# GatorSense/HyperPRI

Measured on AMD Instinct MI355X. Metric: HSI cubes/sec (608x968x238) fwd+bwd, higher is better.
Workload: dtype f32; 1 GPU; CubeNET-64 n_channels=238 HSI 608x968 fp32, per-GPU batch 2, train mode, BCEWithLogits, fwd+bwd; global_batch=2, parallelism=dp1

## Files before the change

### hyperpri_amd/csrc/api.cpp

```cpp
#include "common.h"
#include <string.h>

static thread_local char g_err[256] = "";

int hpri_set_error(int code, const char* msg) {
  strncpy(g_err, msg ? msg : "", sizeof(g_err) - 1);
  g_err[sizeof(g_err) - 1] = 0;
  return code;
}

extern "C" const char* hpri_last_error(void) { return g_err; }
extern "C" int hpri_version(void) { return 100; }

#include <stdlib.h>
#include <atomic>
#include <mutex>
static std::atomic<int> g_opt[8];
static std::once_flag g_opt_once;
static const char* const g_opt_name[8] = {"conv_nbx_min", "wgrad_xcd_min_tiles", "wgrad_xcd_min_strips", "bf16v3_tile_width", "bn_wide_cq", "wgrad_cu_reserve", "wgrad_skip_edge", "wino4_fast_epilogue"};
static const char* const g_opt_env[8] = {"HPRI_NBX_MIN", "HPRI_WGRAD_XCD_MIN", "HPRI_WGRAD_XCD_STRIPS", "HPRI_V3_TILE_WIDTH", "HPRI_BN_WIDE_CQ", "HPRI_WGRAD_CU_RESERVE", "HPRI_WGRAD_SKIP_EDGE", "HPRI_WINO4_FAST_EPILOGUE"};
static const int g_opt_default[8] = {9, 128, 2048, 0, 1, 0, 1, 1};

static void opt_init() {
  for (int i = 0; i < 8; ++i) {
    const char* e = getenv(g_opt_env[i]);
    int v = e ? atoi(e) : g_opt_default[i];
    if (v < 0) v = g_opt_default[i];
    g_opt[i].store(v, std::memory_order_relaxed);
  }
}

int hpri_option(int idx) {
  std::call_once(g_opt_once, opt_init);
  return g_opt[idx].load(std::memory_order_relaxed);
}

extern "C" int hpri_set_option(const char* name, int value) {
  std::call_once(g_opt_once, opt_init);
  for (int i = 0; i < 8; ++i)
    if (name && strcmp(name, g_opt_name[i]) == 0) {
      if (value < 0) return hpri_set_error(HPRI_ERR_ARG, "set_option: value must be >= 0");
      g_opt[i].store(value, std::memory_order_release);
      return HPRI_OK;
    }
  return hpri_set_error(HPRI_ERR_ARG, "set_option: unknown option");
}

static std::atomic<int> g_cus[16];
int hpri_cu_count() {
  int dev = 0;
  if (hipGetDevice(&dev) != hipSuccess || dev < 0 || dev >= 16) return 256;
  int n = g_cus[dev].load(std::memory_order_relaxed);
  if (n > 0) return n;
  if (hipDeviceGetAttribute(&n, hipDeviceAttributeMultiprocessorCount, dev) != hipSuccess || n <= 0) n = 256;
  g_cus[dev].store(n, std::memory_order_relaxed);
  return n;
}

static std::mutex g_q_mutex;
static struct { hipStream_t stream; unsigned* q; unsigned seq; bool used; } g_q[32];

HpriQueueHalves hpri_item_queue_take(hipStream_t stream) {
  std::lock_guard<std::mutex> lock(g_q_mutex);
  for (auto& e : g_q)
// ... 18 lines not shown
  if (queue == nullptr) return HPRI_OK;
  for (auto& e : g_q)
    if (!e.used) { e.stream = stream; e.q = reinterpret_cast<unsigned*>(queue); e.seq = 0; e.used = true; return HPRI_OK; }
  return hpri_set_error(HPRI_ERR_ARG, "set_item_queue: more than 32 streams hold a queue");
}

static thread_local float g_loss_scale = 1.f;
float hpri_loss_scale() { return g_loss_scale; }
extern "C" int hpri_set_loss_scale(float scale) {
  HPRI_REQUIRE(scale > 0.f, "set_loss_scale: the scale must be positive");
  g_loss_scale = scale;
  return HPRI_OK;
}

extern "C" int hpri_get_option(const char* name) {
  for (int i = 0; i < 8; ++i)
    if (name && strcmp(name, g_opt_name[i]) == 0) return hpri_option(i);
  return hpri_set_error(HPRI_ERR_ARG, "get_option: unknown option");
}
```

### hyperpri_amd/csrc/gemm_f32v2.hip

```cpp
#include "common.h"

#define F2_BN 128
#define F2_KC 16
#define F2_A_BYTES (256 * 64)
#define F2_B_BYTES (F2_BN * 64)
#define F2_STAGE_BYTES (F2_A_BYTES + F2_B_BYTES)

struct GemmF2Args {
  const float* x; int x_cs, x_coff;
  const float* wp;
  const float* bias;
  float* y; int y_cs, y_coff, y_cw;
  int N, HW;
  int W, H2, W2, py0, px0, cup;
  int nchunks, Ncols, Ncols_pad;
  int accumulate;
  int tiles_img, ntiles, nb_count, per_xcd;
  int ncu, stagger_cycles;
  unsigned *queue, *queue_clear;
};

struct F2Tile { int img, p0, valid, nb, bx; };

template <int MODE>
__global__ __launch_bounds__(256, 2) void gemm_f32v2_kernel(GemmF2Args a) {
  __shared__ __attribute__((aligned(1024))) unsigned char smem[3 * F2_STAGE_BYTES + 2 * F2_BN * 4 + 16];
  float* bias_lds = reinterpret_cast<float*>(smem + 3 * F2_STAGE_BYTES);
  int* next_lds = reinterpret_cast<int*>(smem + 3 * F2_STAGE_BYTES + 2 * F2_BN * 4);

  const int tid = threadIdx.x, lane = tid & 63, wave = __builtin_amdgcn_readfirstlane(tid >> 6);
  const int li = lane & 31, lh = lane >> 5;
  const int xcd = blockIdx.x & 7, nloc = (int)(gridDim.x >> 3);
  const int items_all = a.ntiles * a.nb_count;
  auto tile_of = [&](int k, F2Tile& t) -> bool {
    if (k >= a.per_xcd) return false;
    const int item = xcd * a.per_xcd + k;
    if (item >= items_all) return false;
    t.bx = item / a.nb_count; t.nb = item - t.bx * a.nb_count;
    t.img = t.bx / a.tiles_img;
    t.p0 = (t.bx - t.img * a.tiles_img) * 256;
    t.valid = min(256, a.HW - t.p0);
    return true;
  };

  constexpr unsigned OOB = HPRI_DMA_OOB;
  unsigned aoff[4], goff[2];
  hpri_rsrc_t rs_a = HPRI_MAKE_RSRC(a.x, 0x7FFFFF00);
  const hpri_rsrc_t rs_b = HPRI_MAKE_RSRC(a.wp, 0x7FFFFF00);
  const int chunk_bytes = a.Ncols_pad * 64;
  const int cpt = MODE == 2 ? (a.cup >> 4) : 1;
  auto setup_dma = [&](const F2Tile& t) {
#pragma unroll
    for (int q = 0; q < 4; ++q) {
      const int pix = (q * 4 + wave) * 16 + (lane >> 2);
      const unsigned sw = (unsigned)(((lane & 3) ^ ((pix >> 2) & 3)) << 2);
      unsigned off = OOB;
// ... 31 lines not shown
  __builtin_amdgcn_sched_barrier(0)
#define F2_DMA_A_AT(bo_, c_, q_) HPRI_LDS_DMA16(rs_a, smem + (bo_) + ((q_) * 4 + wave) * 1024, aoff[q_], a_soff(c_))
#define F2_DMA_B_AT(bo_, c_, q_) HPRI_LDS_DMA16(rs_b, smem + (bo_) + F2_A_BYTES + ((q_) * 4 + wave) * 1024, goff[q_], (c_) * chunk_bytes)
#define F2_ISSUE(buf_, c_)                                                               \
  {                                                                                      \
    _Pragma("unroll") for (int q = 0; q < 2; ++q) F2_DMA_B_AT((buf_) * F2_STAGE_BYTES, c_, q); \
    _Pragma("unroll") for (int q = 0; q < 4; ++q) F2_DMA_A_AT((buf_) * F2_STAGE_BYTES, c_, q); \
  }

  const int fofs0 = li * 64 + (((2 * lh + 0) ^ ((li >> 2) & 3)) << 4);
  const int fofs1 = li * 64 + (((2 * lh + 1) ^ ((li >> 2) & 3)) << 4);
  const int S = a.nchunks;

  F2Tile cur, nxt;
  int k = (int)(blockIdx.x >> 3);
  unsigned* const q = a.queue;
  if (blockIdx.x == 0) hpri_q_clear(a.queue_clear, tid);
  const int nstatic = min(nloc, a.ncu >> 3);
  const bool late_start = (unsigned)(blockIdx.x - a.ncu) < (unsigned)a.ncu;
  unsigned pend = 0u;
  if (q != nullptr && tid == 0) pend = hpri_q_draw(q, xcd, k < nstatic ? 1u : 2u);
  if (late_start && a.stagger_cycles > 0) {
    const long long t0 = (long long)__builtin_amdgcn_s_memtime();
    while ((long long)__builtin_amdgcn_s_memtime() - t0 < (long long)a.stagger_cycles) __builtin_amdgcn_s_sleep(32);
  }
  if (q != nullptr && k >= nstatic) {
    if (tid == 0) { next_lds[0] = nstatic + (int)pend; pend += 1u; }
    __syncthreads();
    k = __builtin_amdgcn_readfirstlane(next_lds[0]);
    __syncthreads();
  }
  bool have = tile_of(k, cur);
  if (!have) return;
  setup_dma(cur);
  float bias_next = 0.f;
  auto load_bias = [&](const F2Tile& t) {
    if (tid < F2_BN) {
      const int col = t.nb * F2_BN + tid;
      const int ch = MODE == 1 ? col % a.cup : col;
      bias_next = (a.bias != nullptr && col < a.Ncols) ? a.bias[ch] : 0.f;
    }
  };
  load_bias(cur);
  F2_ISSUE(0, 0)
  if (S > 1) F2_ISSUE(1, 1)
  int slot = 0;

  while (have) {
    if (tid < F2_BN) bias_lds[slot * F2_BN + tid] = bias_next;
    if (q != nullptr && tid == 0) next_lds[slot] = nstatic + (int)pend;

    f32x16 acc[4][2];
#pragma unroll
    for (int ct = 0; ct < 4; ++ct)
#pragma unroll
      for (int pt = 0; pt < 2; ++pt)
#pragma unroll
        for (int r = 0; r < 16; ++r) acc[ct][pt][r] = 0.f;

    int bo = 0;
    for (int s = 0; s < S; ++s) {
      if (s + 1 < S) F2_WAIT_VM(6); else F2_WAIT_VM(0);
      F2_BARRIER();
      const unsigned char* wb_ = smem + bo + F2_A_BYTES;
      const unsigned char* xb_ = smem + bo + wave * 4096;
      f32x4 wa[4][2], xb[2][2];
#pragma unroll
      for (int ct = 0; ct < 4; ++ct) {
        wa[ct][0] = *reinterpret_cast<const f32x4*>(wb_ + ct * 2048 + fofs0);
        wa[ct][1] = *reinterpret_cast<const f32x4*>(wb_ + ct * 2048 + fofs1);
      }
#pragma unroll
      for (int pt = 0; pt < 2; ++pt) {
        xb[pt][0] = *reinterpret_cast<const f32x4*>(xb_ + pt * 2048 + fofs0);
        xb[pt][1] = *reinterpret_cast<const f32x4*>(xb_ + pt * 2048 + fofs1);
      }
      const bool more_ = s + 2 < S;
      const int bo2 = bo == 0 ? 2 * F2_STAGE_BYTES : bo - F2_STAGE_BYTES;
      __builtin_amdgcn_s_setprio(1);
#pragma unroll
      for (int g = 0; g < 2; ++g)
#pragma unroll
        for (int j = 0; j < 4; ++j) {
#pragma unroll
          for (int ct = 0; ct < 4; ++ct)
#pragma unroll
            for (int pt = 0; pt < 2; ++pt)
              acc[ct][pt] = __builtin_amdgcn_mfma_f32_32x32x2f32(wa[ct][g][j], xb[pt][g][j], acc[ct][pt], 0, 0, 0);
          const int step = g * 4 + j;
          if (more_ && step < 2) { F2_DMA_B_AT(bo2, s + 2, step); }
          if (more_ && step >= 2 && step < 6) { F2_DMA_A_AT(bo2, s + 2, step - 2); }
        }
      __builtin_amdgcn_s_setprio(0);
      bo = bo == 2 * F2_STAGE_BYTES ? 0 : bo + F2_STAGE_BYTES;
    }
    F2_BARRIER();
    if (q != nullptr) k = __builtin_amdgcn_readfirstlane(next_lds[slot]);
    else k += nloc;
    have = tile_of(k, nxt);
    if (have) {
      setup_dma(nxt);
      F2_ISSUE(0, 0)
      if (S > 1) F2_ISSUE(1, 1)
      load_bias(nxt);
      if (q != nullptr && tid == 0) pend = hpri_q_draw(q, xcd, 1u);
    }

#pragma unroll
    for (int pt = 0; pt < 2; ++pt) {
      const int pix = wave * 64 + pt * 32 + li;
      const bool ok = pix < cur.valid;
      const int p = cur.p0 + min(pix, cur.valid - 1);
      long long orow;
      if (MODE == 1) {
        const int yy = p / a.W, xx = p - yy * a.W;
        orow = ((long long)cur.img * a.H2 + a.py0 + 2 * yy) * a.W2 + a.px0 + 2 * xx;
      } else {
        orow = (long long)cur.img * a.HW + p;
      }
      if (MODE != 1 && a.accumulate) {
#pragma unroll
        for (int hh = 0; hh < 2; ++hh) {
// ... 27 lines not shown
          if (MODE == 1) {
            if (ok && col < a.Ncols) {
              const int tap = col / a.cup, co = col - tap * a.cup;
              const long long rr = orow + (long long)((tap >> 1) * a.W2 + (tap & 1));
              *reinterpret_cast<f32x4*>(a.y + rr * a.y_cs + a.y_coff + co) = v;
            }
          } else {
            if (ok && col < a.y_cw) {
#pragma unroll
              for (int e = 0; e < 4; ++e) if (col + e >= a.Ncols) v[e] = 0.f;
              *reinterpret_cast<f32x4*>(a.y + orow * a.y_cs + a.y_coff + col) = v;
            }
          }
        }
    }
    cur = nxt;
    slot ^= 1;
  }
#undef F2_ISSUE
#undef F2_DMA_A_AT
#undef F2_DMA_B_AT
#undef F2_WAIT_VM
#undef F2_BARRIER
}

__global__ void pack_weight_f32k16_kernel(const float* __restrict__ w, float* __restrict__ wp, int mode, int K, int Ncols,
                                          int Ncols_pad, int chunks, int Cup, int src_d1) {
  const size_t total = (size_t)chunks * Ncols_pad * 16;
  for (size_t idx = (size_t)blockIdx.x * blockDim.x + threadIdx.x; idx < total; idx += (size_t)gridDim.x * blockDim.x) {
    const int kk = (int)(idx & 15);
    const size_t r = idx >> 4;
    const int col = (int)(r % Ncols_pad), chunk = (int)(r / Ncols_pad);
    const int k = chunk * 16 + kk;
    float v = 0.f;
    if (k < K && col < Ncols) {
      if (mode == 0) v = w[(size_t)col * src_d1 + k];
      else if (mode == 1) v = w[(size_t)k * src_d1 + col];
      else if (mode == 2) { const int tap = col / Cup, co = col - tap * Cup; v = w[((size_t)k * Cup + co) * 4 + tap]; }
// ... 9 lines not shown
                                       hipStream_t stream) {
  HPRI_REQUIRE(w && wp, "pack_weight_f32k16: null pointer");
  HPRI_REQUIRE(mode >= 0 && mode <= 3 && K > 0 && Ncols > 0 && Ncols_pad >= Ncols && Ncols_pad % 64 == 0, "pack_weight_f32k16: bad arguments");
  HPRI_REQUIRE(mode < 2 || Cup > 0, "pack_weight_f32k16: the transposed-convolution modes need Cup");
  const int chunks = hpri_cdiv(K, 16);
  const size_t total = (size_t)chunks * Ncols_pad * 16;
  int blocks = (int)((total + 255) / 256);
  if (blocks > 4096) blocks = 4096;
  hipLaunchKernelGGL(pack_weight_f32k16_kernel, dim3(blocks), dim3(256), 0, stream, w, wp, mode, K, Ncols, Ncols_pad, chunks, Cup, src_d1);
  HPRI_CHECK_LAUNCH();
  return HPRI_OK;
}

#define F2_STAGGER_CYCLES 8000

static int f2_launch(int mode, const float* x, int x_cs, int x_coff, const float* wp, const float* bias, float* y, int y_cs, int y_coff,
                     int y_cw, int N, long long HW, int W, int H2, int W2, int py0, int px0, int cup, int K_pad, int Ncols,
                     int Ncols_pad, int accumulate, hipStream_t stream) {
  HPRI_REQUIRE(x && wp && y, "gemm_f32v2: null pointer");
  HPRI_REQUIRE(N > 0 && HW > 0 && HW < (1ll << 30), "gemm_f32v2: bad row counts");
  HPRI_REQUIRE(K_pad > 0 && K_pad % 16 == 0, "gemm_f32v2: K_pad must be a positive multiple of 16");
  HPRI_REQUIRE(Ncols > 0 && Ncols_pad % 64 == 0 && Ncols <= Ncols_pad, "gemm_f32v2: Ncols_pad must be a multiple of 64 >= Ncols");
  HPRI_REQUIRE(x_cs % 4 == 0 && x_coff % 4 == 0 && x_cs > 0 && x_cs <= 16384, "gemm_f32v2: row stride / offset must be multiples of 4 (stride <= 16384)");
  HPRI_REQUIRE(((uintptr_t)x & 15) == 0 && ((uintptr_t)wp & 15) == 0 && ((uintptr_t)y & 15) == 0, "gemm_f32v2: pointers must be 16-byte aligned");
  HPRI_REQUIRE(y_cs % 4 == 0 && y_coff % 4 == 0, "gemm_f32v2: the output view must be float4-aligned");
  HPRI_REQUIRE((long long)(K_pad / 16) * Ncols_pad * 64 < 0x7FFFFF00ll, "gemm_f32v2: packed weights exceed 2 GiB");
  GemmF2Args a;
  a.x = x; a.x_cs = x_cs; a.x_coff = x_coff; a.wp = wp; a.bias = bias;
  a.y = y; a.y_cs = y_cs; a.y_coff = y_coff; a.y_cw = y_cw;
  a.N = N; a.HW = (int)HW; a.W = W; a.H2 = H2; a.W2 = W2; a.py0 = py0; a.px0 = px0; a.cup = cup;
  a.nchunks = K_pad / 16; a.Ncols = Ncols; a.Ncols_pad = Ncols_pad; a.accumulate = accumulate & 1;
  if (mode == 0 || mode == 2) {
    HPRI_REQUIRE(y_cw % 4 == 0 && y_cw >= Ncols && y_cw + y_coff <= y_cs, "gemm_f32v2: written width must be a multiple of 4 >= Ncols inside the row stride");
// ... 7 lines not shown
  }
  if (mode == 1) {
    HPRI_REQUIRE(cup % 4 == 0 && Ncols == 4 * cup && !a.accumulate, "gemm_f32v2: depth-to-space needs Cup % 4 == 0, 4*Cup columns and no accumulate");
    HPRI_REQUIRE(x_coff + K_pad <= x_cs && cup + y_coff <= y_cs, "gemm_f32v2: rows narrower than K_pad / Cup channels exceed the output stride");
  }
  if (mode == 2) {
    HPRI_REQUIRE(cup % 16 == 0 && K_pad == 4 * cup && x_coff + cup <= x_cs, "gemm_f32v2: space-to-depth needs Cup % 16 == 0 and K = 4*Cup");
    HPRI_REQUIRE((long long)H2 * W2 * x_cs * 4 < 0x7FFFFF00ll, "gemm_f32v2: one image of the gradient tensor exceeds 2 GiB (32-bit DMA offsets)");
  }
  a.tiles_img = (int)((HW + 255) / 256); a.ntiles = N * a.tiles_img; a.nb_count = (Ncols_pad + F2_BN - 1) / F2_BN;
  const long long items = (long long)a.ntiles * a.nb_count;
  HPRI_REQUIRE(items < (1ll << 28), "gemm_f32v2: too many work items");
  a.per_xcd = (int)((items + 7) / 8);
  a.ncu = hpri_cu_count(); a.stagger_cycles = F2_STAGGER_CYCLES;
  a.queue = a.queue_clear = nullptr;
  int nloc = (2 * a.ncu) / 8;
  if (nloc < 1) nloc = 1;
  if (nloc > a.per_xcd) nloc = a.per_xcd;
  dim3 grid((unsigned)(nloc * 8));
  if (a.per_xcd >= 2 * nloc) { const HpriQueueHalves qh = hpri_item_queue_take(stream); a.queue = qh.use; a.queue_clear = qh.clear; }
  if (mode == 0) hipLaunchKernelGGL(gemm_f32v2_kernel<0>, grid, dim3(256), 0, stream, a);
  else if (mode == 1) hipLaunchKernelGGL(gemm_f32v2_kernel<1>, grid, dim3(256), 0, stream, a);
  else hipLaunchKernelGGL(gemm_f32v2_kernel<2>, grid, dim3(256), 0, stream, a);
  HPRI_CHECK_LAUNCH();
  return HPRI_OK;
}

extern "C" int hpri_gemm_f32v2(const float* x, int x_cs, int x_coff, const float* wp, const float* bias, float* y, int y_cs, int y_coff,
                               int N, long long HW, int K_pad, int Ncols, int Ncols_pad, int y_cw, int accumulate, hipStream_t stream) {
  return f2_launch(0, x, x_cs, x_coff, wp, bias, y, y_cs, y_coff, y_cw, N, HW, 0, 0, 0, 0, 0, 0, K_pad, Ncols, Ncols_pad, accumulate, stream);
}

extern "C" int hpri_convt_fwd_f32v2(const float* x, int x_cs, int x_coff, const float* wp, const float* bias, float* y, int y_cs,
                                    int y_coff, int N, int H, int W, int K_pad, int Cup, int Ncols_pad, int H2, int W2, int py0, int px0,
                                    hipStream_t stream) {
  return f2_launch(1, x, x_cs, x_coff, wp, bias, y, y_cs, y_coff, 0, N, (long long)H * W, W, H2, W2, py0, px0, Cup, K_pad, 4 * Cup, Ncols_pad,
                   0, stream);
}

extern "C" int hpri_convt_dgrad_f32v2(const float* dy, int dy_cs, int dy_coff, const float* wp, float* dx, int dx_cs, int dx_coff, int N,
                                      int H, int W, int Cup, int Cin, int Cin_pad, int dx_cw, int H2, int W2, int py0, int px0,
                                      int accumulate, hipStream_t stream) {
  return f2_launch(2, dy, dy_cs, dy_coff, wp, nullptr, dx, dx_cs, dx_coff, dx_cw, N, (long long)H * W, W, H2, W2, py0, px0, Cup, 4 * Cup, Cin,
                   Cin_pad, accumulate & 1, stream);
}
```

### hyperpri_amd/engine.py

```python
from __future__ import annotations

import contextlib
import ctypes
import threading
import os
import types
from typing import Callable, Dict, List, Optional, Tuple

import torch

from . import _lib

A_DIRECT, A_S2D = 0, 1
E_DIRECT, E_D2S = 0, 1

PRECISIONS = ("fp32", "bf16", "bf16x3", "bf16x6")
LOWP = ("bf16", "bf16x3", "bf16x6")
_SPLIT = {"bf16": 0, "bf16x3": 1, "bf16x6": 2}
DEFAULT_PRECISION = os.environ.get("HPRI_PRECISION", "fp32")

TORCH = "torch"
_CALL = threading.local()


# ... 781 lines not shown
def _pack(w: torch.Tensor, mode: int, K: int, ncols: int, T: int, cup: int, d1: int) -> Tuple[torch.Tensor, int]:
    ncols_pad = _rup(ncols, 64)

    def build():
        global PACK_LAUNCHES
        n = _lib.load().hpri_packed_weight_floats(K, ncols_pad, T)
        wp = torch.empty(n, dtype=torch.float32, device=w.device)
        _lib.call("hpri_pack_weight", _p(w), _p(wp), mode, K, ncols, ncols_pad, T, cup, 0, d1, _stream())
        PACK_LAUNCHES += 1
        return wp
    return _cached_pack(w, ("f32", mode, K, ncols, T, cup, d1), build), ncols_pad


GEMM_F32V2 = True
GEMM_F32V2_DGRAD = False


def _pack_f32k16(w: torch.Tensor, mode: int, K: int, ncols: int, cup: int, d1: int = 0) -> Tuple[torch.Tensor, int]:
    ncols_pad = _rup(ncols, 64)

    def build():
        global PACK_LAUNCHES
        wp = torch.empty(_lib.load().hpri_packed_weight_f32k16_floats(K, ncols_pad), dtype=torch.float32, device=w.device)
        _lib.call("hpri_pack_weight_f32k16", _p(w), _p(wp), mode, K, ncols, ncols_pad, cup, d1, _stream())
        PACK_LAUNCHES += 1
        return wp
    return _cached_pack(w, ("f32k16", mode, K, ncols, cup, d1), build), ncols_pad


def _pack_bf16(w: torch.Tensor, mode: int, K: int, ncols: int, T: int, d1: int, cup: int = 0,
# ... 874 lines not shown
            with _timed("gemm_planes_bf16<convT,s2d>", 2.0 * x1.N * x1.H * x1.W * cin * 4 * cup):
                _lib.call("hpri_convt_dgrad_bf16v3_y16", _p(gpl.buf), gpl.cs, gpl.coff, _p(wpd), gx.ptr, gx.cs, gx.coff, x1.N, x1.H, x1.W,
                          cup, cin, cols_pad, cin, H2, W2, py0, px0, _stream())
        else:
            gx, acc = tp.grad_slot(x1)
            with _timed("gemm_planes_bf16<convT,s2d>", 2.0 * x1.N * x1.H * x1.W * cin * 4 * cup):
                _lib.call("hpri_convt_dgrad_bf16v3", _p(gpl.buf), gpl.cs, gpl.coff, _p(wpd), gx.ptr, gx.cs, gx.coff, x1.N, x1.H, x1.W, cup,
                          cin, cols_pad, gx.cw, H2, W2, py0, px0, int(acc), _stream())
    elif need_dx1:
        gx, acc = tp.grad_slot(x1)
        if bprec in LOWP:
            wpd, cols_pad = _pack_bf16(weight, 3, 4 * cup, cin, 1, cup, cup, split=_SPLIT.get(bprec, 0))
            _conv_launch_bf16(gu, wpd, None, gx, None, x1.N, x1.H, x1.W, 4 * cup, cin, cols_pad, gx.cw, 1,
                              amode=A_S2D, accumulate=int(acc), H2=H2, W2=W2, py0=py0, px0=px0, cup=cup, cin_true=4 * cup,
                              split=_SPLIT.get(bprec, 0))
        elif GEMM_F32V2_DGRAD and cup % 16 == 0 and H2 * W2 * gu.cs * 4 < 0x7FFFFF00 and x1.N * H2 * W2 < (1 << 31):
            wpd, cols_pad = _pack_f32k16(weight, 3, 4 * cup, cin, cup)
            with _timed("gemm_f32v2<convT,s2d>", 2.0 * x1.N * x1.H * x1.W * cin * 4 * cup):
                _lib.call("hpri_convt_dgrad_f32v2", gu.ptr, gu.cs, gu.coff, _p(wpd), gx.ptr, gx.cs, gx.coff, x1.N, x1.H, x1.W, cup, cin, cols_pad,
                          gx.cw, H2, W2, py0, px0, int(acc), _stream())
        else:
            wpd, cols_pad = _pack(weight, 3, 4 * cup, cin, 1, cup, cup)
            _conv_launch(gu, wpd, None, gx, None, x1.N, x1.H, x1.W, 4 * cup, cin, cols_pad, gx.cw, 1,
                         amode=A_S2D, accumulate=int(acc), H2=H2, W2=W2, py0=py0, px0=px0, cup=cup, cin_true=4 * cup)


def _upsample_into(tape: Tape, x1: Act, dst: Act, weight: Optional[torch.Tensor], bias: Optional[torch.Tensor],
                   need_dx1: bool, precision: Optional[str] = None, dst_planes=None) -> bool:
    dev = x1.buf.device
    H2, W2 = dst.H, dst.W
    dY, dX = H2 - 2 * x1.H, W2 - 2 * x1.W
    py0, px0 = dY // 2, dX // 2
    cup = dst.C
    if cup % 4:
        raise RuntimeError("hyperpri_amd: Up: channel counts must be multiples of 4")
    if dY < 0 or dX < 0:
        full = Act.new(x1.N, 2 * x1.H, 2 * x1.W, cup, dev)
        _upsample_into(tape, x1, full, weight, bias, need_dx1, precision)
        _lib.call("hpri_shift_copy", full.ptr, full.cs, full.coff, full.H, full.W, dst.ptr, dst.cs, dst.coff, dst.N, H2, W2,
# ... 31 lines not shown
                              px0 + 2 * x1.W, _stream())
                with _timed("gemm_planes_bf16<convT,d2s+planes>", 2.0 * x1.N * x1.H * x1.W * cin * 4 * cup):
                    _lib.call("hpri_convt_fwd_bf16v3", _p(xp_.buf), xp_.cs, xp_.coff, _p(wp), _p(bias), ctypes.c_void_p(0), 0, 0,
                              _p(pl.buf), pl.cs, pc0, x1.N, x1.H, x1.W, _rup(cin, 32), cup, ncols_pad, H2, W2, py0, px0, _stream())
            else:
                with _timed("conv_fwd_bf16<1,4x1,direct,d2s+planes>", 2.0 * x1.N * x1.H * x1.W * cin * 4 * cup):
                    _lib.call("hpri_convt_fwd_bf16_pl", x1.ptr, x1.cs, x1.coff, _p(wp), _p(bias), ctypes.c_void_p(0), dst.cs, dst.coff,
                              x1.N, x1.H, x1.W, x1.cw, 4 * cup, ncols_pad, H2, W2, py0, px0, cup, _p(pl.buf), pl.cs, pc0, _stream())
            planes_written = True
        elif bf16:
            wp, ncols_pad = _pack_bf16(weight, 2, cin, 4 * cup, 1, cup, cup, split=usplit)
            _conv_launch_bf16(x1, wp, bias, dst, None, x1.N, x1.H, x1.W, x1.cw, 4 * cup, ncols_pad, 4 * cup, 1,
                              epi=E_D2S, H2=H2, W2=W2, py0=py0, px0=px0, cup=cup, cin_true=cin, split=usplit)
        elif GEMM_F32V2 and cin % 16 == 0 and x1.N * H2 * W2 < (1 << 31):
            wp, ncols_pad = _pack_f32k16(weight, 2, cin, 4 * cup, cup)
            with _timed("gemm_f32v2<convT,d2s>", 2.0 * x1.N * x1.H * x1.W * cin * 4 * cup):
                _lib.call("hpri_convt_fwd_f32v2", x1.ptr, x1.cs, x1.coff, _p(wp), _p(bias), dst.ptr, dst.cs, dst.coff, x1.N, x1.H, x1.W, cin,
                          cup, ncols_pad, H2, W2, py0, px0, _stream())
        else:
            wp, ncols_pad = _pack(weight, 2, cin, 4 * cup, 1, cup, cup)
            _conv_launch(x1, wp, bias, dst, None, x1.N, x1.H, x1.W, x1.cw, 4 * cup, ncols_pad, 4 * cup, 1,
                         epi=E_D2S, H2=H2, W2=W2, py0=py0, px0=px0, cup=cup, cin_true=cin)
        del wp
    else:
        if x1.C != cup:
            raise RuntimeError("hyperpri_amd: Up: bilinear upsampling keeps the channel count")
        _lib.call("hpri_upsample2x_fwd", x1.ptr, x1.cs, x1.coff, dst.ptr, dst.cs, dst.coff, x1.N, x1.H, x1.W, H2, W2,
                  py0, px0, cup, _stream())
    if not tape.record:
        return planes_written
    c = types.SimpleNamespace(dst=dst, weight=weight, bias=bias, need_dx1=need_dx1, x1=x1, precision=precision, dev=dev, H2=H2, W2=W2,
                              py0=py0, px0=px0, cup=cup, dY=dY, dX=dX)
    tape.note_params(weight, bias)
# ... 337 lines not shown
```

### include/hyperpri_hip.h

```cpp
#ifndef HYPERPRI_HIP_H
#define HYPERPRI_HIP_H

#include <stddef.h>
#include <hip/hip_runtime_api.h>

#ifdef __cplusplus
extern "C" {
#endif

#define HPRI_OK 0
#define HPRI_ERR_ARG (-1)
#define HPRI_ERR_UNSUPPORTED (-2)
#define HPRI_ERR_WORKSPACE (-3)
#define HPRI_ERR_LAUNCH (-4)

#define HPRI_A_DIRECT 0
#define HPRI_A_S2D 1
#define HPRI_E_DIRECT 0
#define HPRI_E_D2S 1

int hpri_version(void);
int hpri_set_option(const char* name, int value);


// ... 90 lines not shown
                        float* stats, int N, int H, int W, int Cin_pad, int Cout, int Cout_pad, int y_cw, void* y2, int y2_cs,
                        int y2_coff, int y2_c0, int y2_cw, int y2_only, hipStream_t stream);


size_t hpri_packed_weight_f32k16_floats(int K, int Ncols_pad);
int hpri_pack_weight_f32k16(const float* w, float* wp, int mode, int K, int Ncols, int Ncols_pad, int Cup, int src_d1,
                            hipStream_t stream);
int hpri_gemm_f32v2(const float* x, int x_cs, int x_coff, const float* wp, const float* bias, float* y, int y_cs, int y_coff,
                    int N, long long HW, int K_pad, int Ncols, int Ncols_pad, int y_cw, int accumulate, hipStream_t stream);
int hpri_convt_fwd_f32v2(const float* x, int x_cs, int x_coff, const float* wp, const float* bias, float* y, int y_cs,
                         int y_coff, int N, int H, int W, int K_pad, int Cup, int Ncols_pad, int H2, int W2, int py0, int px0,
                         hipStream_t stream);
int hpri_convt_dgrad_f32v2(const float* dy, int dy_cs, int dy_coff, const float* wp, float* dx, int dx_cs, int dx_coff, int N,
                           int H, int W, int Cup, int Cin, int Cin_pad, int dx_cw, int H2, int W2, int py0, int px0,
                           int accumulate, hipStream_t stream);

int hpri_gemm_bf16v3_plan(int N, long long HW, int* stat_tiles);
int hpri_gemm_bf16v3(const void* xp, int x_cs, int x_coff, const void* wp, const float* bias, float* y, int y_cs, int y_coff,
                     void* y16, int y16_cs, int y16_coff, float* stats, int stat_cp, int N, long long HW, int K_pad, int Ncols,
                     int Ncols_pad, int y_cw, int accumulate, hipStream_t stream);
int hpri_convt_fwd_bf16v3(const void* xp, int x_cs, int x_coff, const void* wp, const float* bias, float* y, int y_cs, int y_coff,
                          void* y16, int y16_cs, int y16_coff, int N, int H, int W, int K_pad, int Cup, int Ncols_pad, int H2,
                          int W2, int py0, int px0, hipStream_t stream);
int hpri_convt_dgrad_bf16v3(const void* dyp, int dy_cs, int dy_coff, const void* wp, float* dx, int dx_cs, int dx_coff, int N,
                            int H, int W, int Cup, int Cin, int Cin_pad, int dx_cw, int H2, int W2, int py0, int px0,
                            int accumulate, hipStream_t stream);
int hpri_convt_dgrad_bf16v3_y16(const void* dyp, int dy_cs, int dy_coff, const void* wp, void* dx16, int dx_cs, int dx_coff, int N,
                                int H, int W, int Cup, int Cin, int Cin_pad, int dx_cw, int H2, int W2, int py0, int px0,
                                hipStream_t stream);

// ... 297 lines not shown
```

Baseline: 68.52 cubes/s.

## Add stream-K split-K scheduling with fixup pass to f32v2 transposed-conv GEMMs

Adds a stream-K variant of the f32v2 GEMM. Each workgroup takes a contiguous range of (tile, K-chunk) units, so the last wave of tiles no longer leaves CUs idle. Partial accumulators for tiles split across workgroups go to a workspace, and a separate fixup kernel sums them and applies bias and the output epilogue. The Python engine sends the (1024,512) convT forward and the (1024,512)/(512,256) convT dgrad to this path, which also turns on the f32v2 dgrad kernel for those shapes where it was off before. The costs are extra workspace traffic, an additional launch, and a per-workgroup prefix count of pieces.

```diff
diff --git a/hyperpri_amd/csrc/api.cpp b/hyperpri_amd/csrc/api.cpp
--- a/hyperpri_amd/csrc/api.cpp
+++ b/hyperpri_amd/csrc/api.cpp
@@ -15,14 +15,15 @@
 #include <stdlib.h>
 #include <atomic>
 #include <mutex>
-static std::atomic<int> g_opt[8];
+#define HPRI_NOPT 11
+static std::atomic<int> g_opt[HPRI_NOPT];
 static std::once_flag g_opt_once;
-static const char* const g_opt_name[8] = {"conv_nbx_min", "wgrad_xcd_min_tiles", "wgrad_xcd_min_strips", "bf16v3_tile_width", "bn_wide_cq", "wgrad_cu_reserve", "wgrad_skip_edge", "wino4_fast_epilogue"};
-static const char* const g_opt_env[8] = {"HPRI_NBX_MIN", "HPRI_WGRAD_XCD_MIN", "HPRI_WGRAD_XCD_STRIPS", "HPRI_V3_TILE_WIDTH", "HPRI_BN_WIDE_CQ", "HPRI_WGRAD_CU_RESERVE", "HPRI_WGRAD_SKIP_EDGE", "HPRI_WINO4_FAST_EPILOGUE"};
-static const int g_opt_default[8] = {9, 128, 2048, 0, 1, 0, 1, 1};
+static const char* const g_opt_name[HPRI_NOPT] = {"conv_nbx_min", "wgrad_xcd_min_tiles", "wgrad_xcd_min_strips", "bf16v3_tile_width", "bn_wide_cq", "wgrad_cu_reserve", "wgrad_skip_edge", "wino4_fast_epilogue", "gemm_f32v2_streamk", "gemm_f32v2_workgroups", "plan_cu_count"};
+static const char* const g_opt_env[HPRI_NOPT] = {"HPRI_NBX_MIN", "HPRI_WGRAD_XCD_MIN", "HPRI_WGRAD_XCD_STRIPS", "HPRI_V3_TILE_WIDTH", "HPRI_BN_WIDE_CQ", "HPRI_WGRAD_CU_RESERVE", "HPRI_WGRAD_SKIP_EDGE", "HPRI_WINO4_FAST_EPILOGUE", "HPRI_GEMM_F32V2_STREAMK", "HPRI_GEMM_F32V2_WORKGROUPS", "HPRI_PLAN_CU_COUNT"};
+static const int g_opt_default[HPRI_NOPT] = {9, 128, 2048, 0, 1, 0, 1, 1, 1, 0, 0};
 
 static void opt_init() {
-  for (int i = 0; i < 8; ++i) {
+  for (int i = 0; i < HPRI_NOPT; ++i) {
     const char* e = getenv(g_opt_env[i]);
     int v = e ? atoi(e) : g_opt_default[i];
     if (v < 0) v = g_opt_default[i];
@@ -37,7 +38,7 @@
 
 extern "C" int hpri_set_option(const char* name, int value) {
   std::call_once(g_opt_once, opt_init);
-  for (int i = 0; i < 8; ++i)
+  for (int i = 0; i < HPRI_NOPT; ++i)
     if (name && strcmp(name, g_opt_name[i]) == 0) {
       if (value < 0) return hpri_set_error(HPRI_ERR_ARG, "set_option: value must be >= 0");
       g_opt[i].store(value, std::memory_order_release);
@@ -48,6 +49,8 @@
 
 static std::atomic<int> g_cus[16];
 int hpri_cu_count() {
+  const int planned = hpri_option(10);
+  if (planned > 0) return planned;
   int dev = 0;
   if (hipGetDevice(&dev) != hipSuccess || dev < 0 || dev >= 16) return 256;
   int n = g_cus[dev].load(std::memory_order_relaxed);
@@ -96,7 +99,7 @@
 }
 
 extern "C" int hpri_get_option(const char* name) {
-  for (int i = 0; i < 8; ++i)
+  for (int i = 0; i < HPRI_NOPT; ++i)
     if (name && strcmp(name, g_opt_name[i]) == 0) return hpri_option(i);
   return hpri_set_error(HPRI_ERR_ARG, "get_option: unknown option");
 }
diff --git a/hyperpri_amd/csrc/gemm_f32v2.hip b/hyperpri_amd/csrc/gemm_f32v2.hip
--- a/hyperpri_amd/csrc/gemm_f32v2.hip
+++ b/hyperpri_amd/csrc/gemm_f32v2.hip
@@ -22,8 +22,36 @@
 
 struct F2Tile { int img, p0, valid, nb, bx; };
 
-template <int MODE>
-__global__ __launch_bounds__(256, 2) void gemm_f32v2_kernel(GemmF2Args a) {
+#define F2_SK_MAX_WG 32768
+#define F2_TILE_FLOATS (256 * F2_BN)
+struct GemmF2SK {
+  float* ws;
+  int units, G, per, rem;
+};
+__host__ __device__ static inline int f2_bound(const GemmF2SK& sk, int w) { return w * sk.per + (int)((unsigned)(w * sk.rem) / (unsigned)sk.G); }
+__host__ __device__ static inline int f2_pieces_of(const GemmF2SK& sk, int S, int w) {
+  const int u0 = f2_bound(sk, w), u1 = f2_bound(sk, w + 1);
+  const bool head = u0 % S != 0;
+  const bool tail = u1 % S != 0 && (!head || u0 / S != u1 / S);
+  return (head ? 1 : 0) + (tail ? 1 : 0);
+}
+#ifdef __HIPCC__
+__device__ __forceinline__ int f2_pieces_before(const GemmF2SK& sk, int S, int w, int tid, int* red) {
+  int n = 0;
+  for (int j = tid; j < w; j += 256) n += f2_pieces_of(sk, S, j);
+#pragma unroll
+  for (int off = 32; off > 0; off >>= 1) n += __shfl_xor(n, off);
+  if ((tid & 63) == 0) red[tid >> 6] = n;
+  __syncthreads();
+  n = red[0] + red[1] + red[2] + red[3];
+  __syncthreads();
+  return __builtin_amdgcn_readfirstlane(n);
+}
+#endif
+#define F2_WS_QUAD(ct_, q_, pt_, wave_, lane_) ((((((ct_) * 4 + (q_)) * 2 + (pt_)) * 4 + (wave_)) * 64 + (lane_)) * 4)
+
+template <int MODE, bool SK>
+__device__ __forceinline__ void f2_body(const GemmF2Args& a, const GemmF2SK& sk) {
   __shared__ __attribute__((aligned(1024))) unsigned char smem[3 * F2_STAGE_BYTES + 2 * F2_BN * 4 + 16];
   float* bias_lds = reinterpret_cast<float*>(smem + 3 * F2_STAGE_BYTES);
   int* next_lds = reinterpret_cast<int*>(smem + 3 * F2_STAGE_BYTES + 2 * F2_BN * 4);
@@ -32,14 +60,26 @@
   const int li = lane & 31, lh = lane >> 5;
   const int xcd = blockIdx.x & 7, nloc = (int)(gridDim.x >> 3);
   const int items_all = a.ntiles * a.nb_count;
+  auto item_tile = [&](int item, F2Tile& t) {
+    t.bx = item / a.nb_count; t.nb = item - t.bx * a.nb_count;
+    t.img = t.bx / a.tiles_img;
+    t.p0 = (t.bx - t.img * a.tiles_img) * 256;
+    t.valid = min(256, a.HW - t.p0);
+  };
   auto tile_of = [&](int k, F2Tile& t) -> bool {
     if (k >= a.per_xcd) return false;
     const int item = xcd * a.per_xcd + k;
     if (item >= items_all) return false;
-    t.bx = item / a.nb_count; t.nb = item - t.bx * a.nb_count;
-    t.img = t.bx / a.tiles_img;
-    t.p0 = (t.bx - t.img * a.tiles_img) * 256;
-    t.valid = min(256, a.HW - t.p0);
+    item_tile(item, t);
+    return true;
+  };
+  int u = 0, u_end = 0, wslot = 0;
+  auto seg_of = [&](int uu, F2Tile& t, int& k0, int& k1) -> bool {
+    if (uu >= u_end) return false;
+    const int item = uu / a.nchunks;
+    k0 = uu - item * a.nchunks;
+    k1 = min(a.nchunks, k0 + (u_end - uu));
+    item_tile(item, t);
     return true;
   };
 
@@ -101,7 +141,8 @@
 
   F2Tile cur, nxt;
   int k = (int)(blockIdx.x >> 3);
-  unsigned* const q = a.queue;
+  int kb = 0, ke = S, nkb = 0, nke = S;
+  unsigned* const q = SK ? nullptr : a.queue;
   if (blockIdx.x == 0) hpri_q_clear(a.queue_clear, tid);
   const int nstatic = min(nloc, a.ncu >> 3);
   const bool late_start = (unsigned)(blockIdx.x - a.ncu) < (unsigned)a.ncu;
@@ -117,7 +158,16 @@
     k = __builtin_amdgcn_readfirstlane(next_lds[0]);
     __syncthreads();
   }
-  bool have = tile_of(k, cur);
+  bool have;
+  if (SK) {
+    const int wl = (gridDim.x & 7u) == 0u ? xcd * nloc + k : (int)blockIdx.x;
+    u = f2_bound(sk, wl);
+    u_end = f2_bound(sk, wl + 1);
+    wslot = f2_pieces_before(sk, S, wl, tid, next_lds);
+    have = seg_of(u, cur, kb, ke);
+  } else {
+    have = tile_of(k, cur);
+  }
   if (!have) return;
   setup_dma(cur);
   float bias_next = 0.f;
@@ -129,8 +179,8 @@
     }
   };
   load_bias(cur);
-  F2_ISSUE(0, 0)
-  if (S > 1) F2_ISSUE(1, 1)
+  F2_ISSUE(0, kb)
+  if (ke - kb > 1) F2_ISSUE(1, kb + 1)
   int slot = 0;
 
   while (have) {
@@ -146,8 +196,8 @@
         for (int r = 0; r < 16; ++r) acc[ct][pt][r] = 0.f;
 
     int bo = 0;
-    for (int s = 0; s < S; ++s) {
-      if (s + 1 < S) F2_WAIT_VM(6); else F2_WAIT_VM(0);
+    for (int s = kb; s < ke; ++s) {
+      if (s + 1 < ke) F2_WAIT_VM(6); else F2_WAIT_VM(0);
       F2_BARRIER();
       const unsigned char* wb_ = smem + bo + F2_A_BYTES;
       const unsigned char* xb_ = smem + bo + wave * 4096;
@@ -162,7 +212,7 @@
         xb[pt][0] = *reinterpret_cast<const f32x4*>(xb_ + pt * 2048 + fofs0);
         xb[pt][1] = *reinterpret_cast<const f32x4*>(xb_ + pt * 2048 + fofs1);
       }
-      const bool more_ = s + 2 < S;
+      const bool more_ = s + 2 < ke;
       const int bo2 = bo == 0 ? 2 * F2_STAGE_BYTES : bo - F2_STAGE_BYTES;
       __builtin_amdgcn_s_setprio(1);
 #pragma unroll
@@ -182,17 +232,45 @@
       bo = bo == 2 * F2_STAGE_BYTES ? 0 : bo + F2_STAGE_BYTES;
     }
     F2_BARRIER();
-    if (q != nullptr) k = __builtin_amdgcn_readfirstlane(next_lds[slot]);
-    else k += nloc;
-    have = tile_of(k, nxt);
+    if (SK) {
+      u += ke - kb;
+      have = seg_of(u, nxt, nkb, nke);
+    } else {
+      if (q != nullptr) k = __builtin_amdgcn_readfirstlane(next_lds[slot]);
+      else k += nloc;
+      have = tile_of(k, nxt);
+    }
     if (have) {
       setup_dma(nxt);
-      F2_ISSUE(0, 0)
-      if (S > 1) F2_ISSUE(1, 1)
+      F2_ISSUE(0, nkb)
+      if (nke - nkb > 1) F2_ISSUE(1, nkb + 1)
       load_bias(nxt);
       if (q != nullptr && tid == 0) pend = hpri_q_draw(q, xcd, 1u);
     }
 
+    const bool cut = SK && (kb != 0 || ke != S);
+    if (cut) {
+      const unsigned long long pw = (unsigned long long)(uintptr_t)(sk.ws + (size_t)wslot * F2_TILE_FLOATS);
+      const unsigned wlo = __builtin_amdgcn_readfirstlane((unsigned)pw), whi = __builtin_amdgcn_readfirstlane((unsigned)(pw >> 32));
+      (void)wlo; (void)whi;
+      const hpri_rsrc_t rs_w = HPRI_MAKE_RSRC((((unsigned long long)whi << 32) | wlo), F2_TILE_FLOATS * 4);
+      (void)rs_w;
+      const unsigned woff = (unsigned)F2_WS_QUAD(0, 0, 0, wave, lane) * 4u;
+      (void)woff;
+#pragma unroll
+      for (int ct = 0; ct < 4; ++ct)
+#pragma unroll
+        for (int q = 0; q < 4; ++q)
+#pragma unroll
+          for (int pt = 0; pt < 2; ++pt) {
+            f32x4 v;
+#pragma unroll
+            for (int e = 0; e < 4; ++e) v[e] = acc[ct][pt][4 * q + e];
+            HPRI_BUFFER_STORE_F32X4(v, rs_w, woff, F2_WS_QUAD(ct, q, pt, 0, 0) * 4);
+          }
+      wslot += 1;
+    }
+    if (!cut) {
 #pragma unroll
     for (int pt = 0; pt < 2; ++pt) {
       const int pix = wave * 64 + pt * 32 + li;
@@ -250,7 +328,9 @@
           }
         }
     }
+    }
     cur = nxt;
+    if (SK) { kb = nkb; ke = nke; }
     slot ^= 1;
   }
 #undef F2_ISSUE
@@ -258,6 +338,91 @@
 #undef F2_DMA_B_AT
 #undef F2_WAIT_VM
 #undef F2_BARRIER
+}
+
+template <int MODE>
+__global__ __launch_bounds__(256, 2) void gemm_f32v2_kernel(GemmF2Args a) {
+  GemmF2SK none;
+  none.ws = nullptr; none.units = 0; none.G = 1; none.per = 0; none.rem = 0;
+  f2_body<MODE, false>(a, none);
+}
+
+template <int MODE>
+__global__ __launch_bounds__(256, 2) void gemm_f32v2_kernel_sk(GemmF2Args a, GemmF2SK sk) { f2_body<MODE, true>(a, sk); }
+
+template <int MODE>
+__global__ __launch_bounds__(256) void gemm_f32v2_fixup_kernel(GemmF2Args a, GemmF2SK sk) {
+  const int tid = threadIdx.x, lane = tid & 63, wave = tid >> 6;
+  const int li = lane & 31, lh = lane >> 5;
+  const int S = a.nchunks, G = sk.G;
+  const int w = (int)blockIdx.x + 1;
+  __shared__ int red[4];
+  auto bound = [&](int i) -> int { return f2_bound(sk, i); };
+  const int b = bound(w);
+  if (b % S == 0) return;
+  const int item = b / S, i0 = item * S;
+  const int bp = bound(w - 1);
+  if (bp > i0) return;
+  const int slot0 = f2_pieces_before(sk, S, w - 1, tid, red) + ((bp < i0 && bp % S != 0) ? 1 : 0);
+  int np = 1;
+  for (int j = w; j < G && bound(j) < i0 + S; ++j) ++np;
+  F2Tile t;
+  t.bx = item / a.nb_count; t.nb = item - t.bx * a.nb_count;
+  t.img = t.bx / a.tiles_img;
+  t.p0 = (t.bx - t.img * a.tiles_img) * 256;
+  t.valid = min(256, a.HW - t.p0);
+  const float* const p0_ = sk.ws + (size_t)slot0 * F2_TILE_FLOATS;
+  const int ct = (int)blockIdx.y;
+#pragma unroll
+  for (int pt = 0; pt < 2; ++pt) {
+    const int pix = wave * 64 + pt * 32 + li;
+    const bool ok = pix < t.valid;
+    const int p = t.p0 + min(pix, t.valid - 1);
+    long long orow;
+    if (MODE == 1) {
+      const int yy = p / a.W, xx = p - yy * a.W;
+      orow = ((long long)t.img * a.H2 + a.py0 + 2 * yy) * a.W2 + a.px0 + 2 * xx;
+    } else {
+      orow = (long long)t.img * a.HW + p;
+    }
+    {
+      f32x4 v[4];
+#pragma unroll
+      for (int q = 0; q < 4; ++q) v[q] = *reinterpret_cast<const f32x4*>(p0_ + F2_WS_QUAD(ct, q, pt, wave, lane));
+      for (int pc = 1; pc < np; ++pc)
+#pragma unroll
+        for (int q = 0; q < 4; ++q) {
+          const f32x4 r = *reinterpret_cast<const f32x4*>(p0_ + (size_t)pc * F2_TILE_FLOATS + F2_WS_QUAD(ct, q, pt, wave, lane));
+#pragma unroll
+          for (int e = 0; e < 4; ++e) v[q][e] += r[e];
+        }
+#pragma unroll
+      for (int q = 0; q < 4; ++q) {
+        const int col = t.nb * F2_BN + ct * 32 + 8 * q + 4 * lh;
+        const int tap = MODE == 1 ? col / a.cup : 0, co = col - tap * a.cup;
+        f32x4 o = v[q];
+        if (MODE != 1 && a.accumulate && ok && col < a.y_cw) {
+          const f32x4 old = *reinterpret_cast<const f32x4*>(a.y + orow * a.y_cs + a.y_coff + col);
+#pragma unroll
+          for (int e = 0; e < 4; ++e) o[e] += old[e];
+        }
+#pragma unroll
+        for (int e = 0; e < 4; ++e) o[e] += (a.bias != nullptr && col + e < a.Ncols) ? a.bias[co + e] : 0.f;
+        if (MODE == 1) {
+          if (ok && col < a.Ncols) {
+            const long long rr = orow + (long long)((tap >> 1) * a.W2 + (tap & 1));
+            *reinterpret_cast<f32x4*>(a.y + rr * a.y_cs + a.y_coff + co) = o;
+          }
+        } else {
+          if (ok && col < a.y_cw) {
+#pragma unroll
+            for (int e = 0; e < 4; ++e) if (col + e >= a.Ncols) o[e] = 0.f;
+            *reinterpret_cast<f32x4*>(a.y + orow * a.y_cs + a.y_coff + col) = o;
+          }
+        }
+      }
+    }
+  }
 }
 
 __global__ void pack_weight_f32k16_kernel(const float* __restrict__ w, float* __restrict__ wp, int mode, int K, int Ncols,
@@ -297,9 +462,68 @@
 
 #define F2_STAGGER_CYCLES 8000
 
+struct F2Plan { int use_sk, G, S, pieces, cut_tiles; long long items, units; GemmF2SK sk; };
+
+static int f2_plan(int mode, int N, long long HW, int K_pad, int Ncols_pad, F2Plan& pl) {
+  HPRI_REQUIRE(mode >= 0 && mode <= 2, "gemm_f32v2_plan: mode must be 0, 1 or 2");
+  HPRI_REQUIRE(N > 0 && HW > 0 && HW < (1ll << 30), "gemm_f32v2: bad row counts");
+  HPRI_REQUIRE(K_pad > 0 && K_pad % 16 == 0, "gemm_f32v2: K_pad must be a positive multiple of 16");
+  HPRI_REQUIRE(Ncols_pad > 0 && Ncols_pad % 64 == 0, "gemm_f32v2: Ncols_pad must be a positive multiple of 64");
+  pl.S = K_pad / 16;
+  pl.items = (long long)N * ((HW + 255) / 256) * ((Ncols_pad + F2_BN - 1) / F2_BN);
+  HPRI_REQUIRE(pl.items < (1ll << 28), "gemm_f32v2: too many work items");
+  pl.units = pl.items * pl.S;
+  pl.use_sk = 0; pl.pieces = 0; pl.cut_tiles = 0;
+  const int slots = ((2 * hpri_cu_count()) / 8) * 8;
+  const int forced = hpri_option(9);
+  pl.G = forced > 0 ? forced : slots;
+  if (hpri_option(8) == 0 || pl.G < 1 || pl.G > F2_SK_MAX_WG || pl.units >= (1ll << 31)) return HPRI_OK;
+  if (forced > 0) {
+    pl.use_sk = pl.units >= pl.G;
+  } else {
+    const long long rounds = (pl.items + slots - 1) / slots;
+    pl.use_sk = pl.items * 100 < 90 * rounds * slots && pl.units / pl.G >= 8;
+  }
+  if (!pl.use_sk) return HPRI_OK;
+  pl.sk.ws = nullptr; pl.sk.units = (int)pl.units; pl.sk.G = pl.G;
+  pl.sk.per = (int)(pl.units / pl.G); pl.sk.rem = (int)(pl.units % pl.G);
+  for (int w = 0; w < pl.G; ++w) {
+    pl.pieces += f2_pieces_of(pl.sk, pl.S, w);
+    const int u0 = f2_bound(pl.sk, w);
+    if (w > 0 && u0 % pl.S != 0 && f2_bound(pl.sk, w - 1) <= (u0 / pl.S) * pl.S) pl.cut_tiles += 1;
+  }
+  return HPRI_OK;
+}
+
+extern "C" int hpri_gemm_f32v2_plan(int mode, int N, long long HW, int K_pad, int Ncols_pad, int* use_streamk, int* workgroups,
+                                    size_t* ws_floats) {
+  F2Plan pl;
+  const int rc = f2_plan(mode, N, HW, K_pad, Ncols_pad, pl);
+  if (rc != HPRI_OK) return rc;
+  if (use_streamk) *use_streamk = pl.use_sk;
+  if (workgroups) *workgroups = pl.G;
+  if (ws_floats) *ws_floats = (size_t)pl.pieces * F2_TILE_FLOATS;
+  return HPRI_OK;
+}
+
+extern "C" int hpri_gemm_f32v2_plan_ranges(int mode, int N, long long HW, int K_pad, int Ncols_pad, int cap, long long* unit0, int* piece0) {
+  F2Plan pl;
+  const int rc = f2_plan(mode, N, HW, K_pad, Ncols_pad, pl);
+  if (rc != HPRI_OK) return rc;
+  HPRI_REQUIRE(unit0 && piece0, "gemm_f32v2_plan_ranges: null pointer");
+  HPRI_REQUIRE(pl.use_sk, "gemm_f32v2_plan_ranges: this problem keeps the fixed tiling");
+  HPRI_REQUIRE(cap >= pl.G + 1, "gemm_f32v2_plan_ranges: the tables need workgroups + 1 entries");
+  int np = 0;
+  for (int w = 0; w <= pl.G; ++w) {
+    unit0[w] = f2_bound(pl.sk, w); piece0[w] = np;
+    if (w < pl.G) np += f2_pieces_of(pl.sk, pl.S, w);
+  }
+  return HPRI_OK;
+}
+
 static int f2_launch(int mode, const float* x, int x_cs, int x_coff, const float* wp, const float* bias, float* y, int y_cs, int y_coff,
                      int y_cw, int N, long long HW, int W, int H2, int W2, int py0, int px0, int cup, int K_pad, int Ncols,
-                     int Ncols_pad, int accumulate, hipStream_t stream) {
+                     int Ncols_pad, int accumulate, hipStream_t stream, int ws_given = 0, float* ws = nullptr, size_t ws_floats = 0) {
   HPRI_REQUIRE(x && wp && y, "gemm_f32v2: null pointer");
   HPRI_REQUIRE(N > 0 && HW > 0 && HW < (1ll << 30), "gemm_f32v2: bad row counts");
   HPRI_REQUIRE(K_pad > 0 && K_pad % 16 == 0, "gemm_f32v2: K_pad must be a positive multiple of 16");
@@ -337,6 +561,30 @@
   a.per_xcd = (int)((items + 7) / 8);
   a.ncu = hpri_cu_count(); a.stagger_cycles = F2_STAGGER_CYCLES;
   a.queue = a.queue_clear = nullptr;
+  if (ws_given) {
+    F2Plan pl;
+    const int rc = f2_plan(mode, N, HW, K_pad, Ncols_pad, pl);
+    if (rc != HPRI_OK) return rc;
+    if (pl.use_sk) {
+      if (pl.pieces > 0 && (ws == nullptr || ((uintptr_t)ws & 15) != 0 || ws_floats < (size_t)pl.pieces * F2_TILE_FLOATS))
+        return hpri_set_error(HPRI_ERR_WORKSPACE, "gemm_f32v2: workspace too small or misaligned (hpri_gemm_f32v2_plan)");
+      GemmF2SK sk = pl.sk;
+      sk.ws = ws;
+      const dim3 sgrid((unsigned)pl.G);
+      if (mode == 0) hipLaunchKernelGGL(gemm_f32v2_kernel_sk<0>, sgrid, dim3(256), 0, stream, a, sk);
+      else if (mode == 1) hipLaunchKernelGGL(gemm_f32v2_kernel_sk<1>, sgrid, dim3(256), 0, stream, a, sk);
+      else hipLaunchKernelGGL(gemm_f32v2_kernel_sk<2>, sgrid, dim3(256), 0, stream, a, sk);
+      HPRI_CHECK_LAUNCH();
+      if (pl.cut_tiles > 0) {
+        const dim3 fgrid((unsigned)(pl.G - 1), 4);
+        if (mode == 0) hipLaunchKernelGGL(gemm_f32v2_fixup_kernel<0>, fgrid, dim3(256), 0, stream, a, sk);
+        else if (mode == 1) hipLaunchKernelGGL(gemm_f32v2_fixup_kernel<1>, fgrid, dim3(256), 0, stream, a, sk);
+        else hipLaunchKernelGGL(gemm_f32v2_fixup_kernel<2>, fgrid, dim3(256), 0, stream, a, sk);
+        HPRI_CHECK_LAUNCH();
+      }
+      return HPRI_OK;
+    }
+  }
   int nloc = (2 * a.ncu) / 8;
   if (nloc < 1) nloc = 1;
   if (nloc > a.per_xcd) nloc = a.per_xcd;
@@ -367,3 +615,24 @@
   return f2_launch(2, dy, dy_cs, dy_coff, wp, nullptr, dx, dx_cs, dx_coff, dx_cw, N, (long long)H * W, W, H2, W2, py0, px0, Cup, 4 * Cup, Cin,
                    Cin_pad, accumulate & 1, stream);
 }
+
+extern "C" int hpri_gemm_f32v2_ws(const float* x, int x_cs, int x_coff, const float* wp, const float* bias, float* y, int y_cs, int y_coff,
+                                  int N, long long HW, int K_pad, int Ncols, int Ncols_pad, int y_cw, int accumulate, float* ws,
+                                  size_t ws_floats, hipStream_t stream) {
+  return f2_launch(0, x, x_cs, x_coff, wp, bias, y, y_cs, y_coff, y_cw, N, HW, 0, 0, 0, 0, 0, 0, K_pad, Ncols, Ncols_pad, accumulate, stream, 1,
+                   ws, ws_floats);
+}
+
+extern "C" int hpri_convt_fwd_f32v2_ws(const float* x, int x_cs, int x_coff, const float* wp, const float* bias, float* y, int y_cs,
+                                       int y_coff, int N, int H, int W, int K_pad, int Cup, int Ncols_pad, int H2, int W2, int py0, int px0,
+                                       float* ws, size_t ws_floats, hipStream_t stream) {
+  return f2_launch(1, x, x_cs, x_coff, wp, bias, y, y_cs, y_coff, 0, N, (long long)H * W, W, H2, W2, py0, px0, Cup, K_pad, 4 * Cup, Ncols_pad,
+                   0, stream, 1, ws, ws_floats);
+}
+
+extern "C" int hpri_convt_dgrad_f32v2_ws(const float* dy, int dy_cs, int dy_coff, const float* wp, float* dx, int dx_cs, int dx_coff, int N,
+                                         int H, int W, int Cup, int Cin, int Cin_pad, int dx_cw, int H2, int W2, int py0, int px0,
+                                         int accumulate, float* ws, size_t ws_floats, hipStream_t stream) {
+  return f2_launch(2, dy, dy_cs, dy_coff, wp, nullptr, dx, dx_cs, dx_coff, dx_cw, N, (long long)H * W, W, H2, W2, py0, px0, Cup, 4 * Cup, Cin,
+                   Cin_pad, accumulate & 1, stream, 1, ws, ws_floats);
+}
diff --git a/hyperpri_amd/engine.py b/hyperpri_amd/engine.py
--- a/hyperpri_amd/engine.py
+++ b/hyperpri_amd/engine.py
@@ -819,6 +819,14 @@
 
 GEMM_F32V2 = True
 GEMM_F32V2_DGRAD = False
+F32V2_FWD_ROUTE: Dict[Tuple[int, int], str] = {(1024, 512): "streamk"}
+F32V2_DGRAD_ROUTE: Dict[Tuple[int, int], str] = {(1024, 512): "streamk", (512, 256): "streamk"}
+
+
+def _f32v2_streamk_ws(mode: int, N: int, HW: int, k_pad: int, ncols_pad: int, device) -> Optional[torch.Tensor]:
+    sk = ctypes.c_int(); g = ctypes.c_int(); wsf = ctypes.c_size_t()
+    _lib.call("hpri_gemm_f32v2_plan", mode, N, HW, k_pad, ncols_pad, ctypes.byref(sk), ctypes.byref(g), ctypes.byref(wsf))
+    return _ws(wsf.value, device) if sk.value else None
 
 
 def _pack_f32k16(w: torch.Tensor, mode: int, K: int, ncols: int, cup: int, d1: int = 0) -> Tuple[torch.Tensor, int]:
@@ -1723,15 +1731,30 @@
             _conv_launch_bf16(gu, wpd, None, gx, None, x1.N, x1.H, x1.W, 4 * cup, cin, cols_pad, gx.cw, 1,
                               amode=A_S2D, accumulate=int(acc), H2=H2, W2=W2, py0=py0, px0=px0, cup=cup, cin_true=4 * cup,
                               split=_SPLIT.get(bprec, 0))
-        elif GEMM_F32V2_DGRAD and cup % 16 == 0 and H2 * W2 * gu.cs * 4 < 0x7FFFFF00 and x1.N * H2 * W2 < (1 << 31):
+        elif ((ws := _f32v2_dgrad_route(x1, cin, cup, dev)) is not False and cup % 16 == 0
+              and H2 * W2 * gu.cs * 4 < 0x7FFFFF00 and x1.N * H2 * W2 < (1 << 31)):
             wpd, cols_pad = _pack_f32k16(weight, 3, 4 * cup, cin, cup)
             with _timed("gemm_f32v2<convT,s2d>", 2.0 * x1.N * x1.H * x1.W * cin * 4 * cup):
-                _lib.call("hpri_convt_dgrad_f32v2", gu.ptr, gu.cs, gu.coff, _p(wpd), gx.ptr, gx.cs, gx.coff, x1.N, x1.H, x1.W, cup, cin, cols_pad,
-                          gx.cw, H2, W2, py0, px0, int(acc), _stream())
+                if ws is not None:
+                    _lib.call("hpri_convt_dgrad_f32v2_ws", gu.ptr, gu.cs, gu.coff, _p(wpd), gx.ptr, gx.cs, gx.coff, x1.N, x1.H, x1.W, cup, cin,
+                              cols_pad, gx.cw, H2, W2, py0, px0, int(acc), _p(ws), ws.numel(), _stream())
+                else:
+                    _lib.call("hpri_convt_dgrad_f32v2", gu.ptr, gu.cs, gu.coff, _p(wpd), gx.ptr, gx.cs, gx.coff, x1.N, x1.H, x1.W, cup, cin,
+                              cols_pad, gx.cw, H2, W2, py0, px0, int(acc), _stream())
         else:
             wpd, cols_pad = _pack(weight, 3, 4 * cup, cin, 1, cup, cup)
             _conv_launch(gu, wpd, None, gx, None, x1.N, x1.H, x1.W, 4 * cup, cin, cols_pad, gx.cw, 1,
                          amode=A_S2D, accumulate=int(acc), H2=H2, W2=W2, py0=py0, px0=px0, cup=cup, cin_true=4 * cup)
+
+
+def _f32v2_dgrad_route(x1: Act, cin: int, cup: int, device):
+    route = "gemm" if GEMM_F32V2_DGRAD else (F32V2_DGRAD_ROUTE.get((cin, cup)) if GEMM_F32V2 else None)
+    if route == "gemm":
+        return None
+    if route == "streamk" and cup % 16 == 0:
+        ws = _f32v2_streamk_ws(2, x1.N, x1.H * x1.W, 4 * cup, _rup(cin, 64), device)
+        return ws if ws is not None else False
+    return False
 
 
 def _upsample_into(tape: Tape, x1: Act, dst: Act, weight: Optional[torch.Tensor], bias: Optional[torch.Tensor],
@@ -1793,9 +1816,14 @@
                               epi=E_D2S, H2=H2, W2=W2, py0=py0, px0=px0, cup=cup, cin_true=cin, split=usplit)
         elif GEMM_F32V2 and cin % 16 == 0 and x1.N * H2 * W2 < (1 << 31):
             wp, ncols_pad = _pack_f32k16(weight, 2, cin, 4 * cup, cup)
+            ws = _f32v2_streamk_ws(1, x1.N, x1.H * x1.W, cin, ncols_pad, dev) if F32V2_FWD_ROUTE.get((cin, cup)) == "streamk" else None
             with _timed("gemm_f32v2<convT,d2s>", 2.0 * x1.N * x1.H * x1.W * cin * 4 * cup):
-                _lib.call("hpri_convt_fwd_f32v2", x1.ptr, x1.cs, x1.coff, _p(wp), _p(bias), dst.ptr, dst.cs, dst.coff, x1.N, x1.H, x1.W, cin,
-                          cup, ncols_pad, H2, W2, py0, px0, _stream())
+                if ws is not None:
+                    _lib.call("hpri_convt_fwd_f32v2_ws", x1.ptr, x1.cs, x1.coff, _p(wp), _p(bias), dst.ptr, dst.cs, dst.coff, x1.N, x1.H, x1.W,
+                              cin, cup, ncols_pad, H2, W2, py0, px0, _p(ws), ws.numel(), _stream())
+                else:
+                    _lib.call("hpri_convt_fwd_f32v2", x1.ptr, x1.cs, x1.coff, _p(wp), _p(bias), dst.ptr, dst.cs, dst.coff, x1.N, x1.H, x1.W,
+                              cin, cup, ncols_pad, H2, W2, py0, px0, _stream())
         else:
             wp, ncols_pad = _pack(weight, 2, cin, 4 * cup, 1, cup, cup)
             _conv_launch(x1, wp, bias, dst, None, x1.N, x1.H, x1.W, x1.cw, 4 * cup, ncols_pad, 4 * cup, 1,
diff --git a/include/hyperpri_hip.h b/include/hyperpri_hip.h
--- a/include/hyperpri_hip.h
+++ b/include/hyperpri_hip.h
@@ -128,6 +128,18 @@
 int hpri_convt_dgrad_f32v2(const float* dy, int dy_cs, int dy_coff, const float* wp, float* dx, int dx_cs, int dx_coff, int N,
                            int H, int W, int Cup, int Cin, int Cin_pad, int dx_cw, int H2, int W2, int py0, int px0,
                            int accumulate, hipStream_t stream);
+int hpri_gemm_f32v2_plan(int mode, int N, long long HW, int K_pad, int Ncols_pad, int* use_streamk, int* workgroups,
+                         size_t* ws_floats);
+int hpri_gemm_f32v2_plan_ranges(int mode, int N, long long HW, int K_pad, int Ncols_pad, int cap, long long* unit0, int* piece0);
+int hpri_gemm_f32v2_ws(const float* x, int x_cs, int x_coff, const float* wp, const float* bias, float* y, int y_cs, int y_coff,
+                       int N, long long HW, int K_pad, int Ncols, int Ncols_pad, int y_cw, int accumulate, float* ws,
+                       size_t ws_floats, hipStream_t stream);
+int hpri_convt_fwd_f32v2_ws(const float* x, int x_cs, int x_coff, const float* wp, const float* bias, float* y, int y_cs,
+                            int y_coff, int N, int H, int W, int K_pad, int Cup, int Ncols_pad, int H2, int W2, int py0, int px0,
+                            float* ws, size_t ws_floats, hipStream_t stream);
+int hpri_convt_dgrad_f32v2_ws(const float* dy, int dy_cs, int dy_coff, const float* wp, float* dx, int dx_cs, int dx_coff, int N,
+                              int H, int W, int Cup, int Cin, int Cin_pad, int dx_cw, int H2, int W2, int py0, int px0,
+                              int accumulate, float* ws, size_t ws_floats, hipStream_t stream);
 
 int hpri_gemm_bf16v3_plan(int N, long long HW, int* stat_tiles);
 int hpri_gemm_bf16v3(const void* xp, int x_cs, int x_coff, const void* wp, const float* bias, float* y, int y_cs, int y_coff,
```

Result: no change. 68.89 cubes/s, median of 6 (+0.5%).
